# mahdi-slh/DeformContact

Measured on NVIDIA B200. Metric: train_step_graphs_per_sec, higher is better.
Workload: dtype fp32

## Files before the change

### deformcontact_b200/csrc/gemm_tc2.cu

```cuda
#include <cuda.h>
#include <stdlib.h>
#include <string.h>

#include <vector>

#include "common.cuh"

namespace dcb {
namespace {

constexpr int T2_BM = 128, T2_BN = 128, T2_BK = 32;
constexpr int T2_STAGES = 3;
constexpr int T2_THREADS = 512;
constexpr int T2_TILE_BYTES = T2_BM * T2_BK * 4;
constexpr int T2_STAGE_BYTES = 4 * T2_TILE_BYTES;
constexpr int T2_EPI_ROW = 20;
constexpr int T2_EPI_WARP_FLOATS = 32 * T2_EPI_ROW;
constexpr int T2_SMEM_BYTES = T2_STAGES * T2_STAGE_BYTES + 8 * T2_EPI_WARP_FLOATS * 4 + 256 + 1024;
constexpr int T2_DRAIN_KB = 4;
constexpr int T2_DRAIN_KB_SHORT = 4;
constexpr int T2_SHORT_KB = 16;
constexpr int T2_PART_KB = 8;
constexpr int T2_MAX_KPARTS = 64;

struct alignas(64) T2Problem {
  CUtensorMap mapA, mapB;
  CUtensorMap mapC, mapE;
  float* C;
  long long ldc;
  int M, N, kb_total, n_chunks;
  const float* E;
  const float* rowv;
  long long lde;
  int pad[2];
};

struct T2Params {
  const T2Problem* batch;
  const int* item_off;
  int n_problems;
  int nseg;
  int kb_seg[4];
  int kb_total;
  int M, N;
  int m_tiles, n_chunks, k_parts, kb_per_part, items;
  int a_mn, b_mn;
  int drain_kb;
  float* C;
  long long ldc;
  const float* bias;
  int relu, accumulate;
  float* partial;
  int pair;
  int raw_hi;
  int lo_rn;
  float comp;
  int tepi;
};

__device__ __forceinline__ uint32_t smem_u32(const void* p) { return (uint32_t)__cvta_generic_to_shared(p); }
__device__ __forceinline__ void mbar_init(uint32_t bar, uint32_t count) {
  asm volatile("mbarrier.init.shared::cta.b64 [%0], %1;" ::"r"(bar), "r"(count));
}
__device__ __forceinline__ void mbar_arrive(uint32_t bar) {
  asm volatile("mbarrier.arrive.shared::cta.b64 _, [%0];" ::"r"(bar) : "memory");
}
__device__ __forceinline__ void mbar_expect_tx(uint32_t bar, uint32_t bytes) {
  asm volatile("mbarrier.arrive.expect_tx.shared::cta.b64 _, [%0], %1;" ::"r"(bar), "r"(bytes) : "memory");
}
__device__ __forceinline__ void mbar_wait(uint32_t bar, uint32_t parity) {
  asm volatile(
      "{\n\t"
      ".reg .pred p;\n\t"
      "WAIT_%=:\n\t"
      "mbarrier.try_wait.parity.shared::cta.b64 p, [%0], %1;\n\t"
      "@p bra DONE_%=;\n\t"
      "bra WAIT_%=;\n\t"
      "DONE_%=:\n\t"
      "}" ::"r"(bar), "r"(parity)
      : "memory");
}
__device__ __forceinline__ void tma_load_2d(uint32_t dst, const CUtensorMap* map, uint32_t bar, int c0, int c1) {
  asm volatile(
      "cp.async.bulk.tensor.2d.shared::cluster.global.mbarrier::complete_tx::bytes [%0], [%1, {%3, %4}], [%2];" ::"r"(dst),
      "l"(map), "r"(bar), "r"(c0), "r"(c1)
      : "memory");
}
__device__ __forceinline__ void tma_store_2d(const CUtensorMap* map, uint32_t src, int c0, int c1) {
  asm volatile("cp.async.bulk.tensor.2d.global.shared::cta.bulk_group [%0, {%2, %3}], [%1];" ::"l"(map), "r"(src), "r"(c0), "r"(c1)
               : "memory");
}
__device__ __forceinline__ uint64_t l2_evict_first_policy() {
  uint64_t pol;
  asm volatile("createpolicy.fractional.L2::evict_first.b64 %0, 1.0;" : "=l"(pol));
  return pol;
}
__device__ __forceinline__ void tma_store_2d_hint(const CUtensorMap* map, uint32_t src, int c0, int c1, uint64_t pol) {
  asm volatile("cp.async.bulk.tensor.2d.global.shared::cta.bulk_group.L2::cache_hint [%0, {%2, %3}], [%1], %4;" ::"l"(map), "r"(src),
               "r"(c0), "r"(c1), "l"(pol)
               : "memory");
}
__device__ __forceinline__ void tma_load_2d_hint(uint32_t dst, const CUtensorMap* map, uint32_t bar, int c0, int c1, uint64_t pol) {
  asm volatile(
      "cp.async.bulk.tensor.2d.shared::cluster.global.mbarrier::complete_tx::bytes.L2::cache_hint [%0], [%1, {%3, %4}], [%2], %5;" ::"r"(dst),
      "l"(map), "r"(bar), "r"(c0), "r"(c1), "l"(pol)
      : "memory");
}
__device__ __forceinline__ void bulk_commit() { asm volatile("cp.async.bulk.commit_group;" ::: "memory"); }
__device__ __forceinline__ void bulk_wait_read0() { asm volatile("cp.async.bulk.wait_group.read 0;" ::: "memory"); }
__device__ __forceinline__ void bulk_wait0() { asm volatile("cp.async.bulk.wait_group 0;" ::: "memory"); }
__device__ __forceinline__ void tensormap_acquire(const CUtensorMap* map) {
  asm volatile("fence.proxy.tensormap::generic.acquire.sys [%0], 128;" ::"l"(map) : "memory");
}
__device__ __forceinline__ void umma_tf32(uint32_t d_tmem, uint64_t adesc, uint64_t bdesc, uint32_t idesc, uint32_t accum) {
  asm volatile(
      "{\n\t"
      ".reg .pred p;\n\t"
      "setp.ne.b32 p, %4, 0;\n\t"
      "tcgen05.mma.cta_group::1.kind::tf32 [%0], %1, %2, %3, p;\n\t"
      "}" ::"r"(d_tmem),
      "l"(adesc), "l"(bdesc), "r"(idesc), "r"(accum)
      : "memory");
}
__device__ __forceinline__ void umma_commit(uint32_t bar) {
  asm volatile("tcgen05.commit.cta_group::1.mbarrier::arrive::one.shared::cluster.b64 [%0];" ::"r"(bar) : "memory");
}
__device__ __forceinline__ uint32_t cluster_ctarank() {
  uint32_t r;
  asm volatile("mov.u32 %0, %%cluster_ctarank;" : "=r"(r));
  return r;
}
__device__ __forceinline__ void cluster_sync_all() {
  asm volatile("barrier.cluster.arrive.release.aligned;" ::: "memory");
  asm volatile("barrier.cluster.wait.acquire.aligned;" ::: "memory");
  __syncthreads();
}
__device__ __forceinline__ void mbar_arrive_rank(uint32_t bar, uint32_t rank) {
  uint32_t remote;
  asm volatile("mapa.shared::cluster.u32 %0, %1, %2;" : "=r"(remote) : "r"(bar), "r"(rank));
  asm volatile("mbarrier.arrive.shared::cluster.b64 _, [%0];" ::"r"(remote) : "memory");
}
__device__ __forceinline__ void umma2_tf32(uint32_t d_tmem, uint64_t adesc, uint64_t bdesc, uint32_t idesc, uint32_t accum) {
  asm volatile(
      "{\n\t"
      ".reg .pred p;\n\t"
      "setp.ne.b32 p, %4, 0;\n\t"
      "tcgen05.mma.cta_group::2.kind::tf32 [%0], %1, %2, %3, p;\n\t"
      "}" ::"r"(d_tmem),
      "l"(adesc), "l"(bdesc), "r"(idesc), "r"(accum)
      : "memory");
}
__device__ __forceinline__ void umma_commit2(uint32_t bar) {
  asm volatile("tcgen05.commit.cta_group::2.mbarrier::arrive::one.shared::cluster.multicast::cluster.b64 [%0], %1;" ::"r"(bar),
               "h"((unsigned short)3)
               : "memory");
}
__device__ __forceinline__ void tc_fence_before() { asm volatile("tcgen05.fence::before_thread_sync;" ::: "memory"); }
__device__ __forceinline__ void tc_fence_after() { asm volatile("tcgen05.fence::after_thread_sync;" ::: "memory"); }

__device__ __forceinline__ uint64_t desc_kmajor(uint32_t saddr) {
  uint64_t d = 0;
  d |= (uint64_t)((saddr & 0x3FFFF) >> 4);
  d |= (uint64_t)1 << 16;
  d |= (uint64_t)(1024 >> 4) << 32;
  d |= (uint64_t)1 << 46;
  d |= (uint64_t)2 << 61;
  return d;
}
__device__ __forceinline__ uint64_t desc_mnmajor(uint32_t saddr) {
  uint64_t d = 0;
  d |= (uint64_t)((saddr & 0x3FFFF) >> 4);
  d |= (uint64_t)((4096 >> 4) & 0x3FFF) << 16;
  d |= (uint64_t)((512 >> 4) & 0x3FFF) << 32;
  d |= (uint64_t)1 << 46;
  d |= (uint64_t)1 << 61;
  return d;
}

#define T2_TMEM_LD32(R, ADDR)                                                                                            \
  asm volatile(                                                                                                         \
      "tcgen05.ld.sync.aligned.32x32b.x32.b32 "                                                                         \
      "{%0, %1, %2, %3, %4, %5, %6, %7, %8, %9, %10, %11, %12, %13, %14, %15, %16, %17, %18, %19, %20, %21, %22, %23, " \
      "%24, %25, %26, %27, %28, %29, %30, %31}, [%32];"                                                                 \
      : "=r"(R[0]), "=r"(R[1]), "=r"(R[2]), "=r"(R[3]), "=r"(R[4]), "=r"(R[5]), "=r"(R[6]), "=r"(R[7]), "=r"(R[8]),    \
        "=r"(R[9]), "=r"(R[10]), "=r"(R[11]), "=r"(R[12]), "=r"(R[13]), "=r"(R[14]), "=r"(R[15]), "=r"(R[16]),         \
        "=r"(R[17]), "=r"(R[18]), "=r"(R[19]), "=r"(R[20]), "=r"(R[21]), "=r"(R[22]), "=r"(R[23]), "=r"(R[24]),        \
        "=r"(R[25]), "=r"(R[26]), "=r"(R[27]), "=r"(R[28]), "=r"(R[29]), "=r"(R[30]), "=r"(R[31])                       \
      : "r"(ADDR))

struct T2Item {
  int m0, n0, part, kb0, kb1;
  int M, N;
  float* C;
  long long ldc;
  const CUtensorMap *mapA, *mapB;
  const CUtensorMap *mapC, *mapE;
  const float *E, *rowv;
  long long lde;
};
__device__ __forceinline__ T2Item t2_item(const T2Params& p, int w, int& pidx, int rank = 0) {
  T2Item it;
  if (p.batch) {
    while (w >= p.item_off[pidx + 1]) ++pidx;
    const T2Problem* q = p.batch + pidx;
    const int local = w - p.item_off[pidx];
    const int nch = q->n_chunks;
    it.part = 0;
    it.n0 = (local % nch) * T2_BN;
    it.m0 = (p.pair ? (local / nch) * 2 + rank : (local / nch)) * T2_BM;
    it.kb0 = 0;
    it.kb1 = q->kb_total;
    it.M = q->M; it.N = q->N; it.C = q->C; it.ldc = q->ldc;
    it.mapA = &q->mapA; it.mapB = &q->mapB;
    it.mapC = &q->mapC; it.mapE = &q->mapE;
    it.E = q->E; it.rowv = q->rowv; it.lde = q->lde;
    return it;
  }
  it.part = w % p.k_parts;
  const int mn = w / p.k_parts;
  it.n0 = (mn % p.n_chunks) * T2_BN;
  it.m0 = (p.pair ? (mn / p.n_chunks) * 2 + rank : (mn / p.n_chunks)) * T2_BM;
  it.kb0 = it.part * p.kb_per_part;
  it.kb1 = min(p.kb_total, it.kb0 + p.kb_per_part);
  it.M = p.M; it.N = p.N; it.C = p.C; it.ldc = p.ldc;
  it.mapA = nullptr; it.mapB = nullptr;
  it.mapC = nullptr; it.mapE = nullptr;
  it.E = nullptr; it.rowv = nullptr; it.lde = 0;
  return it;
}

template <bool PAIR, bool TEPI>
__global__ void __launch_bounds__(T2_THREADS, 1)
gemm_tc2_kernel(const __grid_constant__ CUtensorMap mapA0, const __grid_constant__ CUtensorMap mapA1,
                const __grid_constant__ CUtensorMap mapA2, const __grid_constant__ CUtensorMap mapA3,
                const __grid_constant__ CUtensorMap mapB0, const __grid_constant__ CUtensorMap mapB1,
                const __grid_constant__ CUtensorMap mapB2, const __grid_constant__ CUtensorMap mapB3,
                const __grid_constant__ CUtensorMap mapC0, const T2Params p) {
  static_assert(PAIR || !TEPI, "the TMA epilogue exists for CTA pairs only");
  extern __shared__ uint8_t smem_raw[];
  const uint32_t base = (smem_u32(smem_raw) + 1023u) & ~1023u;
  uint8_t* base_ptr = smem_raw + (base - smem_u32(smem_raw));
  constexpr int NST = PAIR ? (TEPI ? 3 : 4) : T2_STAGES;
  constexpr int STB = PAIR ? 3 * T2_TILE_BYTES : T2_STAGE_BYTES;
  constexpr int RING = NST * STB;
  constexpr int EPI_WARP_BYTES = TEPI ? 8192 : T2_EPI_WARP_FLOATS * 4;
  constexpr int B_OFF = 2 * T2_TILE_BYTES;
  constexpr int BLO_OFF = PAIR ? B_OFF + T2_TILE_BYTES / 2 : B_OFF + T2_TILE_BYTES;
  static_assert(RING + 8 * EPI_WARP_BYTES + 256 + 1024 <= T2_SMEM_BYTES, "shared memory carve");
  static_assert(TEPI || RING == T2_STAGES * T2_STAGE_BYTES, "stage ring size");
  float* epi_stage = reinterpret_cast<float*>(base_ptr + RING);
  const uint32_t bar_base = base + RING + 8 * EPI_WARP_BYTES;
  auto ebar = [&](int slot) { return bar_base + 160u + 8u * slot; };
  auto full_bar = [&](int s) { return bar_base + 8u * s; };
  auto xform_bar = [&](int s) { return bar_base + 32u + 8u * s; };
  auto empty_bar = [&](int s) { return bar_base + 64u + 8u * s; };
  auto tfull_bar = [&](int j) { return bar_base + 96u + 8u * j; };
  auto tempty_bar = [&](int j) { return bar_base + 112u + 8u * j; };
  volatile uint32_t* tmem_ptr_smem = reinterpret_cast<volatile uint32_t*>(base_ptr + RING + 8 * EPI_WARP_BYTES + 144);

  const int warp = threadIdx.x >> 5, lane = threadIdx.x & 31;
  const int rank = PAIR ? (int)cluster_ctarank() : 0;
  const int w0 = PAIR ? (int)(blockIdx.x >> 1) : (int)blockIdx.x;
  const int wstep = PAIR ? (int)(gridDim.x >> 1) : (int)gridDim.x;

  if (threadIdx.x == 0) {
    for (int s = 0; s < NST; ++s) {
      mbar_init(full_bar(s), 1);
      mbar_init(xform_bar(s), PAIR ? 8 : 128);
      mbar_init(empty_bar(s), 1);
    }
    for (int j = 0; j < 2; ++j) {
      mbar_init(tfull_bar(j), 1);
      mbar_init(tempty_bar(j), PAIR ? 16 : 256);
    }
    if (TEPI)
      for (int sl = 0; sl < 8; ++sl) mbar_init(ebar(sl), 1);
    asm volatile("fence.mbarrier_init.release.cluster;" ::: "memory");
  }
  if (warp == 2) {
    if (PAIR) {
      asm volatile("tcgen05.alloc.cta_group::2.sync.aligned.shared::cta.b32 [%0], %1;" ::"r"(smem_u32((const void*)tmem_ptr_smem)),
                   "r"(512u)
                   : "memory");
      asm volatile("tcgen05.relinquish_alloc_permit.cta_group::2.sync.aligned;" ::: "memory");
    } else {
      asm volatile("tcgen05.alloc.cta_group::1.sync.aligned.shared::cta.b32 [%0], %1;" ::"r"(smem_u32((const void*)tmem_ptr_smem)),
                   "r"(512u)
                   : "memory");
      asm volatile("tcgen05.relinquish_alloc_permit.cta_group::1.sync.aligned;" ::: "memory");
    }
  }
  tc_fence_before();
  if (PAIR) cluster_sync_all(); else __syncthreads();
  tc_fence_after();
  const uint32_t tmem_base = *tmem_ptr_smem;

  if (warp == 0) {
    if (lane == 0) {
      const CUtensorMap* mA[4] = {&mapA0, &mapA1, &mapA2, &mapA3};
      const CUtensorMap* mB[4] = {&mapB0, &mapB1, &mapB2, &mapB3};
      int it = 0, pidx = 0, fenced = -1;
      for (int w = w0; w < p.items; w += wstep) {
        const T2Item item = t2_item(p, w, pidx, rank);
        if (p.batch) {
          mA[0] = item.mapA; mB[0] = item.mapB;
          if (fenced != pidx) {
            tensormap_acquire(item.mapA);
            tensormap_acquire(item.mapB);
            fenced = pidx;
          }
        }
        int seg = 0, seg_kb0 = 0;
        for (int kb = item.kb0; kb < item.kb1; ++kb, ++it) {
          if (!p.batch)
            while (kb >= seg_kb0 + p.kb_seg[seg]) { seg_kb0 += p.kb_seg[seg]; ++seg; }
          const int k0 = (kb - seg_kb0) * T2_BK;
          const int st = it % NST;
          const uint32_t ph = (it / NST) & 1;
          mbar_wait(empty_bar(st), ph ^ 1);
          const uint32_t sbase = base + st * STB;
          mbar_expect_tx(full_bar(st), PAIR ? T2_TILE_BYTES + T2_TILE_BYTES / 2 : 2 * T2_TILE_BYTES);
          if (p.a_mn) {
#pragma unroll
            for (int c = 0; c < 4; ++c) tma_load_2d(sbase + c * 4096, mA[seg], full_bar(st), item.m0 + c * 32, k0);
          } else {
            tma_load_2d(sbase, mA[seg], full_bar(st), k0, item.m0);
          }
          if (PAIR) {
            const int nb0 = item.n0 + rank * (T2_BN / 2);
            if (p.b_mn) {
#pragma unroll
              for (int c = 0; c < 2; ++c) tma_load_2d(sbase + 2 * T2_TILE_BYTES + c * 4096, mB[seg], full_bar(st), nb0 + c * 32, k0);
            } else {
              tma_load_2d(sbase + 2 * T2_TILE_BYTES, mB[seg], full_bar(st), k0, nb0);
            }
          } else if (p.b_mn) {
#pragma unroll
            for (int c = 0; c < 4; ++c) tma_load_2d(sbase + 2 * T2_TILE_BYTES + c * 4096, mB[seg], full_bar(st), item.n0 + c * 32, k0);
          } else {
            tma_load_2d(sbase + 2 * T2_TILE_BYTES, mB[seg], full_bar(st), k0, item.n0);
          }
        }
      }
    }
  } else if (warp == 1) {
    if (lane == 0 && rank == 0) {
      const uint32_t idesc = (1u << 4) | (2u << 7) | (2u << 10) | ((uint32_t)p.a_mn << 15) | ((uint32_t)p.b_mn << 16) |
                             ((uint32_t)(T2_BN >> 3) << 17) | ((uint32_t)(T2_BM >> 4) << 24);
      const uint32_t a_adv = p.a_mn ? (1024u >> 4) : (32u >> 4), b_adv = p.b_mn ? (1024u >> 4) : (32u >> 4);
      const uint32_t idesc256 = (idesc & ~(0x3Fu << 17)) | ((uint32_t)(2 * T2_BN >> 3) << 17);
      const uint32_t idesc_pair = (idesc & ~(0x1Fu << 24)) | ((uint32_t)(2 * T2_BM >> 4) << 24);
      int it = 0, chain = 0, pidx = 0;
      for (int w = w0; w < p.items; w += wstep) {
        const T2Item item = t2_item(p, w, pidx, rank);
        for (int kc0 = item.kb0; kc0 < item.kb1; kc0 += p.drain_kb, ++chain) {
          const int kc1 = min(item.kb1, kc0 + p.drain_kb);
          const int j = chain & 1;
          const uint32_t d_main = tmem_base + (uint32_t)(2 * T2_BN * j), d_cross = d_main + (uint32_t)T2_BN;
          mbar_wait(tempty_bar(j), ((chain >> 1) & 1) ^ 1);
          tc_fence_after();
          for (int kb = kc0; kb < kc1; ++kb, ++it) {
            const int st = it % NST;
            const uint32_t ph = (it / NST) & 1;
            mbar_wait(full_bar(st), ph);
            mbar_wait(xform_bar(st), ph);
            tc_fence_after();
            const uint32_t sbase = base + st * STB;
            const uint64_t a_hi = p.a_mn ? desc_mnmajor(sbase) : desc_kmajor(sbase);
            const uint64_t a_lo = p.a_mn ? desc_mnmajor(sbase + T2_TILE_BYTES) : desc_kmajor(sbase + T2_TILE_BYTES);
            const uint64_t b_hi = p.b_mn ? desc_mnmajor(sbase + 2 * T2_TILE_BYTES) : desc_kmajor(sbase + 2 * T2_TILE_BYTES);
            if (PAIR) {
              const uint64_t b_lo = p.b_mn ? desc_mnmajor(sbase + BLO_OFF) : desc_kmajor(sbase + BLO_OFF);
#pragma unroll
              for (int kk = 0; kk < T2_BK / 8; ++kk) {
                const uint64_t aa = (uint64_t)(kk * a_adv), bb = (uint64_t)(kk * b_adv);
                const uint32_t acc = (kb > kc0 || kk > 0) ? 1u : 0u;
                umma2_tf32(d_main, a_hi + aa, b_hi + bb, idesc_pair, acc);
                umma2_tf32(d_cross, a_hi + aa, b_lo + bb, idesc_pair, acc);
                umma2_tf32(d_cross, a_lo + aa, b_hi + bb, idesc_pair, 1u);
              }
              umma_commit2(empty_bar(st));
            } else {
#pragma unroll
            for (int kk = 0; kk < T2_BK / 8; ++kk) {
              const uint64_t aa = (uint64_t)(kk * a_adv), bb = (uint64_t)(kk * b_adv);
              const uint32_t acc = (kb > kc0 || kk > 0) ? 1u : 0u;
              umma_tf32(d_main, a_hi + aa, b_hi + bb, idesc256, acc);
              umma_tf32(d_cross, a_lo + aa, b_hi + bb, idesc, 1u);
            }
            umma_commit(empty_bar(st));
            }
          }
          if (PAIR) umma_commit2(tfull_bar(j)); else umma_commit(tfull_bar(j));
        }
      }
    }
  } else if (warp >= 8 && warp < 12) {
    const int t = threadIdx.x - 256;
    const uint32_t rb = p.lo_rn ? 0x1000u : 0u;
    int it = 0, pidx = 0;
    for (int w = w0; w < p.items; w += wstep) {
      const T2Item item = t2_item(p, w, pidx, rank);
      for (int kb = item.kb0; kb < item.kb1; ++kb, ++it) {
        const int st = it % NST;
        const uint32_t ph = (it / NST) & 1;
        mbar_wait(full_bar(st), ph);
        uint4* a = reinterpret_cast<uint4*>(base_ptr + st * STB);
        uint4* b = reinterpret_cast<uint4*>(base_ptr + st * STB + B_OFF);
        constexpr int LO = T2_TILE_BYTES / 16;
        constexpr int LO_B = (BLO_OFF - B_OFF) / 16;
#pragma unroll
        for (int i = 0; i < 2 * T2_TILE_BYTES / 16 / 128; ++i) {
          if (PAIR && (i & 1) && (i >> 1) >= T2_TILE_BYTES / 32 / 128) continue;
          uint4* src = (i & 1) ? b : a;
          const int idx = t + (i >> 1) * 128;
          const uint4 v = src[idx];
          const uint4 h = make_uint4(v.x & 0xFFFFE000u, v.y & 0xFFFFE000u, v.z & 0xFFFFE000u, v.w & 0xFFFFE000u);
          uint4 l;
          l.x = __float_as_uint(__uint_as_float(v.x) - __uint_as_float(h.x)) + rb;
          l.y = __float_as_uint(__uint_as_float(v.y) - __uint_as_float(h.y)) + rb;
          l.z = __float_as_uint(__uint_as_float(v.z) - __uint_as_float(h.z)) + rb;
          l.w = __float_as_uint(__uint_as_float(v.w) - __uint_as_float(h.w)) + rb;
          if (!p.raw_hi) src[idx] = h;
          src[idx + ((i & 1) ? LO_B : LO)] = l;
        }
        asm volatile("fence.proxy.async.shared::cta;" ::: "memory");
        if (PAIR) {
          __syncwarp();
          if (lane == 0) mbar_arrive_rank(xform_bar(st), 0);
        } else {
          mbar_arrive(xform_bar(st));
        }
      }
    }
  } else if (warp >= 4) {
    const int q = warp & 3;
    const int half = warp >= 12 ? 1 : 0;
    float* stg = epi_stage + ((half * 4) + q) * T2_EPI_WARP_FLOATS;
    const uint32_t lane_addr = tmem_base + ((uint32_t)(q * 32) << 16) + (uint32_t)(half * 64);
    int chain = 0, pidx = 0;
    const int slot = half * 4 + q;
    const uint32_t ebuf = base + RING + slot * 8192;
    uint8_t* ebuf_ptr = base_ptr + RING + slot * 8192;
    uint32_t eph = 0;
    int efenced = -1;
    const bool ehint = TEPI && (p.tepi & 2);
    const uint64_t epol = ehint ? l2_evict_first_policy() : 0ull;
    for (int w = w0; w < p.items; w += wstep) {
      const T2Item item = t2_item(p, w, pidx, rank);
      const bool vec_ok = ((item.ldc & 3) == 0) && ((reinterpret_cast<uintptr_t>(item.C) & 15) == 0) &&
                          (!p.bias || (reinterpret_cast<uintptr_t>(p.bias) & 15) == 0) && ((item.N & 3) == 0 || p.k_parts == 1);
      float acc[64];
#pragma unroll
      for (int i = 0; i < 64; ++i) acc[i] = 0.f;
      const CUtensorMap* mC = TEPI ? (p.batch ? item.mapC : &mapC0) : nullptr;
      const int ecol0 = item.n0 + half * 64, erow0 = item.m0 + q * 32;
      if (TEPI) {
        if (lane == 0) {
          bulk_wait_read0();
          if (p.batch && efenced != pidx) {
            tensormap_acquire(item.mapC);
            if (item.E != nullptr) tensormap_acquire(item.mapE);
            efenced = pidx;
          }
          if (item.E != nullptr) {
            mbar_expect_tx(ebar(slot), 8192);
            if (ehint) {
              tma_load_2d_hint(ebuf, item.mapE, ebar(slot), ecol0, erow0, epol);
              tma_load_2d_hint(ebuf + 4096, item.mapE, ebar(slot), ecol0 + 32, erow0, epol);
            } else {
              tma_load_2d(ebuf, item.mapE, ebar(slot), ecol0, erow0);
              tma_load_2d(ebuf + 4096, item.mapE, ebar(slot), ecol0 + 32, erow0);
            }
          }
        }
        __syncwarp();
      }
      if (!TEPI && item.E != nullptr) {
        auto prefetch_block = [&](const T2Item& it2) {
          const int prow = it2.m0 + q * 32 + lane;
          const int pcol = it2.n0 + half * 64;
          if (it2.E != nullptr && prow < it2.M && pcol < it2.N) {
            const float* pe = it2.E + (long long)prow * it2.lde + pcol;
            asm volatile("prefetch.global.L2 [%0];" ::"l"(pe));
            if (pcol + 32 < it2.N) asm volatile("prefetch.global.L2 [%0];" ::"l"(pe + 32));
            if (pcol + 63 < it2.N) asm volatile("prefetch.global.L2 [%0];" ::"l"(pe + 63));
          }
        };
        if (w == w0) prefetch_block(item);
        if (w + wstep < p.items) {
          int pidx2 = pidx;
          prefetch_block(t2_item(p, w + wstep, pidx2, rank));
        }
      }
      for (int kc0 = item.kb0; kc0 < item.kb1; kc0 += p.drain_kb, ++chain) {
        const int j = chain & 1;
        mbar_wait(tfull_bar(j), (chain >> 1) & 1);
        tc_fence_after();
        const uint32_t cbase = lane_addr + (uint32_t)(2 * T2_BN * j);
        const float comp = 1.0f + p.comp * (float)(4 * (min(item.kb1, kc0 + p.drain_kb) - kc0));
        uint32_t r[32];
#pragma unroll
        for (int part = 0; part < 4; ++part) {
          T2_TMEM_LD32(r, cbase + (uint32_t)((part >> 1) * T2_BN + (part & 1) * 32));
          asm volatile("tcgen05.wait::ld.sync.aligned;" ::: "memory");
          if (part == 3) {
            tc_fence_before();
            if (PAIR) {
              __syncwarp();
              if (lane == 0) mbar_arrive_rank(tempty_bar(j), 0);
            } else {
              mbar_arrive(tempty_bar(j));
            }
          }
          if (part < 2) {
#pragma unroll
            for (int i = 0; i < 32; ++i) acc[(part & 1) * 32 + i] = fmaf(__uint_as_float(r[i]), comp, acc[(part & 1) * 32 + i]);
          } else {
#pragma unroll
            for (int i = 0; i < 32; ++i) acc[(part & 1) * 32 + i] += __uint_as_float(r[i]);
          }
        }
      }
      if (TEPI) {
        const int row = erow0 + lane;
        float d = 0.f;
        if (item.E != nullptr) {
          if (row < item.M) d = __ldg(item.rowv + row);
          mbar_wait(ebar(slot), eph);
          eph ^= 1;
        }
        const float* bias = p.bias;
        const bool bias_vec = bias && ((reinterpret_cast<uintptr_t>(bias) & 15) == 0);
#pragma unroll
        for (int b = 0; b < 2; ++b) {
#pragma unroll
          for (int c = 0; c < 8; ++c) {
            float4* cell = reinterpret_cast<float4*>(ebuf_ptr + b * 4096 + lane * 128 + ((c ^ (lane & 7)) << 4));
            float4 v = make_float4(acc[b * 32 + c * 4], acc[b * 32 + c * 4 + 1], acc[b * 32 + c * 4 + 2], acc[b * 32 + c * 4 + 3]);
            if (bias) {
              const int col = ecol0 + b * 32 + c * 4;
              if (bias_vec && col + 3 < item.N) {
                const float4 bv = __ldg(reinterpret_cast<const float4*>(bias + col));
                v.x += bv.x; v.y += bv.y; v.z += bv.z; v.w += bv.w;
              } else {
                if (col < item.N) v.x += __ldg(bias + col);
                if (col + 1 < item.N) v.y += __ldg(bias + col + 1);
                if (col + 2 < item.N) v.z += __ldg(bias + col + 2);
                if (col + 3 < item.N) v.w += __ldg(bias + col + 3);
              }
            }
            if (item.E != nullptr) {
              const float4 e = *cell;
              v.x = e.x * (v.x - d); v.y = e.y * (v.y - d); v.z = e.z * (v.z - d); v.w = e.w * (v.w - d);
            }
            if (p.relu) { v.x = fmaxf(v.x, 0.f); v.y = fmaxf(v.y, 0.f); v.z = fmaxf(v.z, 0.f); v.w = fmaxf(v.w, 0.f); }
            *cell = v;
          }
        }
        asm volatile("fence.proxy.async.shared::cta;" ::: "memory");
        __syncwarp();
        if (lane == 0) {
          if (ehint) {
            tma_store_2d_hint(mC, ebuf, ecol0, erow0, epol);
            tma_store_2d_hint(mC, ebuf + 4096, ecol0 + 32, erow0, epol);
          } else {
            tma_store_2d(mC, ebuf, ecol0, erow0);
            tma_store_2d(mC, ebuf + 4096, ecol0 + 32, erow0);
          }
          bulk_commit();
        }
        continue;
      }
      const bool to_slab = p.k_parts > 1;
      float* outp = to_slab ? p.partial + (size_t)item.part * (size_t)item.M * item.N : item.C;
      const long long ldo = to_slab ? (long long)item.N : item.ldc;
      const bool add_c = !to_slab && p.accumulate;
      const bool do_relu = !to_slab && p.relu;
      const float* bias = to_slab ? nullptr : p.bias;
      const int row0 = item.m0 + q * 32;
      if (item.E != nullptr && vec_ok && !add_c && !do_relu && !bias && (item.N & 3) == 0 && (item.lde & 3) == 0 &&
          (reinterpret_cast<uintptr_t>(item.E) & 15) == 0) {
        const int c4 = (lane >> 3) * 4;
        const int rsub = lane & 7;
        const int colbase = item.n0 + half * 64 + c4;
        const float* erow = item.E + (long long)(row0 + rsub) * item.lde + colbase;
        float* orow = outp + (long long)(row0 + rsub) * ldo + colbase;
        float4 xa[4], xb[4];
        float dv[4];
#pragma unroll
        for (int it4 = 0; it4 < 4; ++it4) dv[it4] = (row0 + it4 * 8 + rsub < item.M) ? __ldg(item.rowv + row0 + it4 * 8 + rsub) : 0.f;
        auto load_group = [&](float4 (&x)[4], int g) {
#pragma unroll
          for (int it4 = 0; it4 < 4; ++it4) {
            x[it4] = make_float4(0.f, 0.f, 0.f, 0.f);
            if (row0 + it4 * 8 + rsub < item.M && colbase + g * 16 < item.N)
              x[it4] = __ldcs(reinterpret_cast<const float4*>(erow + (long long)(it4 * 8) * item.lde + g * 16));
          }
        };
        load_group(xa, 0);
#pragma unroll
        for (int g = 0; g < 4; ++g) {
#pragma unroll
          for (int jv = 0; jv < 16; jv += 4)
            *reinterpret_cast<float4*>(stg + lane * T2_EPI_ROW + jv) = make_float4(acc[g * 16 + jv], acc[g * 16 + jv + 1], acc[g * 16 + jv + 2], acc[g * 16 + jv + 3]);
          __syncwarp();
          if (g + 1 < 4) { if (g & 1) load_group(xa, g + 1); else load_group(xb, g + 1); }
#pragma unroll
          for (int it4 = 0; it4 < 4; ++it4) {
            const int rr = it4 * 8 + rsub;
            if (row0 + rr < item.M && colbase + g * 16 < item.N) {
              float4 v = *reinterpret_cast<const float4*>(stg + rr * T2_EPI_ROW + c4);
              const float4 e = (g & 1) ? xb[it4] : xa[it4];
              const float d = dv[it4];
              v.x = e.x * (v.x - d); v.y = e.y * (v.y - d); v.z = e.z * (v.z - d); v.w = e.w * (v.w - d);
              __stcs(reinterpret_cast<float4*>(orow + (long long)(it4 * 8) * ldo + g * 16), v);
            }
          }
          __syncwarp();
        }
        continue;
      }
#pragma unroll
      for (int g = 0; g < 4; ++g) {
#pragma unroll
        for (int jv = 0; jv < 16; jv += 4)
          *reinterpret_cast<float4*>(stg + lane * T2_EPI_ROW + jv) = make_float4(acc[g * 16 + jv], acc[g * 16 + jv + 1], acc[g * 16 + jv + 2], acc[g * 16 + jv + 3]);
        __syncwarp();
        const int c4 = (lane >> 3) * 4;
        const int col = item.n0 + half * 64 + g * 16 + c4;
        if (vec_ok && col + 3 < item.N) {
          const float4 bv = bias ? *reinterpret_cast<const float4*>(bias + col) : make_float4(0.f, 0.f, 0.f, 0.f);
#pragma unroll
          for (int it4 = 0; it4 < 4; ++it4) {
            const int rr = it4 * 8 + (lane & 7);
            const int row = row0 + rr;
            if (row < item.M) {
              float4 v = *reinterpret_cast<const float4*>(stg + rr * T2_EPI_ROW + c4);
              v.x += bv.x; v.y += bv.y; v.z += bv.z; v.w += bv.w;
              if (item.E) {
                const float d = item.rowv[row];
                const float* ep = item.E + (long long)row * item.lde + col;
                float4 e4;
                if (((item.lde & 3) == 0) && ((reinterpret_cast<uintptr_t>(item.E) & 15) == 0)) e4 = *reinterpret_cast<const float4*>(ep);
                else e4 = make_float4(ep[0], ep[1], ep[2], ep[3]);
                v.x = e4.x * (v.x - d); v.y = e4.y * (v.y - d); v.z = e4.z * (v.z - d); v.w = e4.w * (v.w - d);
              }
              float4* dst = reinterpret_cast<float4*>(outp + (long long)row * ldo + col);
              if (add_c) { const float4 o = *dst; v.x += o.x; v.y += o.y; v.z += o.z; v.w += o.w; }
              if (do_relu) { v.x = fmaxf(v.x, 0.f); v.y = fmaxf(v.y, 0.f); v.z = fmaxf(v.z, 0.f); v.w = fmaxf(v.w, 0.f); }
              *dst = v;
            }
          }
        } else {
          for (int it4 = 0; it4 < 4; ++it4) {
            const int rr = it4 * 8 + (lane & 7);
            const int row = row0 + rr;
            for (int e = 0; e < 4; ++e) {
              if (row < item.M && col + e < item.N) {
                float v = stg[rr * T2_EPI_ROW + c4 + e] + (bias ? bias[col + e] : 0.f);
                if (item.E) v = item.E[(long long)row * item.lde + col + e] * (v - item.rowv[row]);
                float* dst = outp + (long long)row * ldo + col + e;
                if (add_c) v += *dst;
                if (do_relu) v = fmaxf(v, 0.f);
                *dst = v;
              }
            }
          }
        }
        __syncwarp();
      }
    }
  }

  if (TEPI && warp >= 4 && !(warp >= 8 && warp < 12) && lane == 0) bulk_wait0();
  tc_fence_before();
  if (PAIR) cluster_sync_all(); else __syncthreads();
  if (warp == 2) {
    tc_fence_after();
    if (PAIR) asm volatile("tcgen05.dealloc.cta_group::2.sync.aligned.b32 %0, %1;" ::"r"(tmem_base), "r"(512u) : "memory");
    else asm volatile("tcgen05.dealloc.cta_group::1.sync.aligned.b32 %0, %1;" ::"r"(tmem_base), "r"(512u) : "memory");
  }
}

__global__ void t2_reduce_kernel(const float* __restrict__ partial, int parts, long long MN, int N, float* __restrict__ C,
                                 long long ldc, const float* __restrict__ bias, int relu, int accumulate) {
  const long long idx = blockIdx.x * (long long)blockDim.x + threadIdx.x;
  if (idx >= MN) return;
  const long long m = idx / N;
  const int n = (int)(idx % N);
  float s = 0.f;
  for (int z = 0; z < parts; ++z) s += partial[(size_t)z * MN + idx];
  if (bias) s += bias[n];
  float* dst = C + m * ldc + n;
  if (accumulate) s += *dst;
  if (relu) s = fmaxf(s, 0.f);
  *dst = s;
}

typedef CUresult (*EncodeFn2)(CUtensorMap*, CUtensorMapDataType, cuuint32_t, void*, const cuuint64_t*, const cuuint64_t*,
                              const cuuint32_t*, const cuuint32_t*, CUtensorMapInterleave, CUtensorMapSwizzle,
                              CUtensorMapL2promotion, CUtensorMapFloatOOBfill);
EncodeFn2 get_encode2() {
  static EncodeFn2 fn = nullptr;
  if (!fn) {
    void* sym = nullptr;
    cudaDriverEntryPointQueryResult qres;
    if (cudaGetDriverEntryPoint("cuTensorMapEncodeTiled", &sym, cudaEnableDefault, &qres) == cudaSuccess &&
        qres == cudaDriverEntryPointSuccess)
      fn = reinterpret_cast<EncodeFn2>(sym);
  }
  return fn;
}

int make_map2(CUtensorMap* map, const float* ptr, uint64_t inner, uint64_t rows, uint64_t ld_elems, uint32_t box_rows,
              CUtensorMapSwizzle swz) {
  EncodeFn2 enc = get_encode2();
  DC_REQUIRE(enc, DC_ECUDA, "gemm_tc2: cuTensorMapEncodeTiled not available");
  cuuint64_t gdim[2] = {inner, rows};
  cuuint64_t gstr[1] = {ld_elems * 4};
  cuuint32_t box[2] = {T2_BK, box_rows};
  cuuint32_t estr[2] = {1, 1};
  CUresult r = enc(map, CU_TENSOR_MAP_DATA_TYPE_FLOAT32, 2, const_cast<float*>(ptr), gdim, gstr, box, estr,
                   CU_TENSOR_MAP_INTERLEAVE_NONE, swz, CU_TENSOR_MAP_L2_PROMOTION_L2_128B, CU_TENSOR_MAP_FLOAT_OOB_FILL_NONE);
  DC_REQUIRE(r == CUDA_SUCCESS, DC_ECUDA, "gemm_tc2: cuTensorMapEncodeTiled failed (%d)", (int)r);
  return DC_OK;
}

int t2_drain_kb(int64_t kb_total) {
  static int d_long = -1, d_short = -1;
  if (d_long < 0) {
    const char* e = getenv("DCB200_DRAIN_KB");
    d_long = (e && atoi(e) > 0) ? atoi(e) : T2_DRAIN_KB;
    const char* es = getenv("DCB200_DRAIN_KB_SHORT");
    d_short = (es && atoi(es) > 0) ? atoi(es) : T2_DRAIN_KB_SHORT;
  }
  return kb_total <= T2_SHORT_KB ? (d_short < d_long ? d_short : d_long) : d_long;
}

void t2_numerics(T2Params& p) {
  static int lo_rn = -1;
  static float comp = -1.f;
  if (lo_rn < 0) {
    const char* e = getenv("DCB200_T2_LO_RN");
    lo_rn = e ? (e[0] == '1') : 1;
    const char* c = getenv("DCB200_T2_COMP");
    comp = c ? (float)atof(c) : 2.6e-8f;
  }
  p.lo_rn = lo_rn;
  p.comp = comp;
}

int t2_pair() {
  static int pair = -1;
  if (pair < 0) {
    const char* e = getenv("DCB200_T2_PAIR");
    pair = e ? (e[0] == '1') : 1;
  }
  return pair;
}

int t2_tepi_mode() {
  static int mode = -1;
  if (mode < 0) {
    const char* e = getenv("DCB200_T2_TEPI");
    mode = e ? atoi(e) : 3;
  }
  return mode;
}
bool t2_tepi_ok(int pair, int64_t kb_max, int k_parts, int accumulate) {
  const int mode = t2_tepi_mode();
  return pair && mode > 0 && k_parts == 1 && !accumulate && (mode > 1 || kb_max <= T2_SHORT_KB);
}
bool t2_tepi_operand_ok(const float* ptr, int64_t ld) { return ptr && (ld & 3) == 0 && (reinterpret_cast<uintptr_t>(ptr) & 15) == 0; }

int t2_launch(const CUtensorMap* mA, const CUtensorMap* mB, const CUtensorMap& mC, const T2Params& p, cudaStream_t st) {
  static DeviceOnce attr_set;
  if (attr_set.first()) {
    DC_CUDA(cudaFuncSetAttribute(gemm_tc2_kernel<false, false>, cudaFuncAttributeMaxDynamicSharedMemorySize, T2_SMEM_BYTES));
    DC_CUDA(cudaFuncSetAttribute(gemm_tc2_kernel<true, false>, cudaFuncAttributeMaxDynamicSharedMemorySize, T2_SMEM_BYTES));
    DC_CUDA(cudaFuncSetAttribute(gemm_tc2_kernel<true, true>, cudaFuncAttributeMaxDynamicSharedMemorySize, T2_SMEM_BYTES));
  }
  if (!p.pair) {
    const int grid = p.items < sm_count() ? p.items : sm_count();
    gemm_tc2_kernel<false, false><<<grid, T2_THREADS, T2_SMEM_BYTES, st>>>(mA[0], mA[1], mA[2], mA[3], mB[0], mB[1], mB[2], mB[3], mC, p);
  } else {
    const int pairs = p.items < sm_count() / 2 ? p.items : sm_count() / 2;
    cudaLaunchConfig_t cfg{};
    cfg.gridDim = dim3((unsigned)(2 * pairs));
    cfg.blockDim = dim3(T2_THREADS);
    cfg.dynamicSmemBytes = T2_SMEM_BYTES;
    cfg.stream = st;
    cudaLaunchAttribute at[1];
    at[0].id = cudaLaunchAttributeClusterDimension;
    at[0].val.clusterDim.x = 2; at[0].val.clusterDim.y = 1; at[0].val.clusterDim.z = 1;
    cfg.attrs = at;
    cfg.numAttrs = 1;
    if (p.tepi) DC_CUDA(cudaLaunchKernelEx(&cfg, gemm_tc2_kernel<true, true>, mA[0], mA[1], mA[2], mA[3], mB[0], mB[1], mB[2], mB[3], mC, p));
    else DC_CUDA(cudaLaunchKernelEx(&cfg, gemm_tc2_kernel<true, false>, mA[0], mA[1], mA[2], mA[3], mB[0], mB[1], mB[2], mB[3], mC, p));
  }
  DC_LAUNCH_CHECK();
  return DC_OK;
}

int t2_k_parts(int64_t M, int64_t N, int64_t kb_total) {
  const int64_t mn = cdiv(M, T2_BM) * cdiv(N, T2_BN);
  if (mn >= sm_count()) return 1;
  int64_t parts = sm_count() / mn;
  const int64_t max_parts = kb_total / T2_PART_KB;
  if (parts > max_parts) parts = max_parts;
  if (parts > T2_MAX_KPARTS) parts = T2_MAX_KPARTS;
  return parts < 1 ? 1 : (int)parts;
}
}

bool gemm_tc2_supported(const dc_gemm_seg* segs, int nseg, int transA, int transB, int64_t M, int64_t N) {
  if (nseg < 1 || nseg > 4 || M < 1 || N < 1 || M >= (1ll << 31) || N >= (1ll << 31)) return false;
  if (nseg > 1 && (transA || !transB)) return false;
  for (int s = 0; s < nseg; ++s) {
    if (segs[s].K <= 0 || segs[s].K >= (1ll << 31)) return false;
    if (segs[s].lda % 4 != 0 || segs[s].ldb % 4 != 0) return false;
    if ((reinterpret_cast<uintptr_t>(segs[s].A) & 15) || (reinterpret_cast<uintptr_t>(segs[s].B) & 15)) return false;
  }
  return true;
}

size_t gemm_tc2_workspace_bytes(int64_t M, int64_t N, int64_t Ktot) {
  const int parts = t2_k_parts(M, N, cdiv(Ktot, T2_BK));
  return parts > 1 ? align_up((size_t)parts * M * N * sizeof(float), 256) + 256 : 0;
}

int gemm_tc2(const dc_gemm_seg* segs, int nseg, int transA, int transB, int64_t M, int64_t N, float* C, int64_t ldc,
             const float* bias, int relu, int accumulate, void* workspace, size_t workspace_bytes, cudaStream_t st) {
  DC_REQUIRE(gemm_tc2_supported(segs, nseg, transA, transB, M, N), DC_ENOSUP, "gemm_tc2: layout not supported by the tcgen05 path");
  T2Params p{};
  p.nseg = nseg;
  p.a_mn = transA ? 1 : 0;
  p.b_mn = transB ? 0 : 1;
  p.pair = t2_pair();
  const uint32_t b_box_rows = p.pair ? T2_BN / 2 : T2_BN;
  CUtensorMap mA[4], mB[4];
  int64_t ktot = 0;
  for (int s = 0; s < 4; ++s) {
    const int ss = s < nseg ? s : 0;
    const uint64_t K = (uint64_t)segs[ss].K;
    if (transA) {
      if (int rc = make_map2(&mA[s], segs[ss].A, (uint64_t)M, K, (uint64_t)segs[ss].lda, 32, CU_TENSOR_MAP_SWIZZLE_128B_ATOM_32B)) return rc;
    } else {
      if (int rc = make_map2(&mA[s], segs[ss].A, K, (uint64_t)M, (uint64_t)segs[ss].lda, T2_BM, CU_TENSOR_MAP_SWIZZLE_128B)) return rc;
    }
    if (transB) {
      if (int rc = make_map2(&mB[s], segs[ss].B, K, (uint64_t)N, (uint64_t)segs[ss].ldb, b_box_rows, CU_TENSOR_MAP_SWIZZLE_128B)) return rc;
    } else {
      if (int rc = make_map2(&mB[s], segs[ss].B, (uint64_t)N, K, (uint64_t)segs[ss].ldb, 32, CU_TENSOR_MAP_SWIZZLE_128B_ATOM_32B)) return rc;
    }
    p.kb_seg[s] = s < nseg ? (int)cdiv(segs[s].K, T2_BK) : (1 << 30);
    if (s < nseg) ktot += cdiv(segs[s].K, T2_BK);
  }
  p.kb_total = (int)ktot;
  p.M = (int)M; p.N = (int)N;
  p.m_tiles = (int)cdiv(M, T2_BM);
  p.n_chunks = (int)cdiv(N, T2_BN);
  p.k_parts = t2_k_parts(M, N, p.kb_total);
  p.kb_per_part = (int)(cdiv(cdiv(p.kb_total, p.k_parts), T2_PART_KB) * T2_PART_KB);
  p.k_parts = (int)cdiv(p.kb_total, p.kb_per_part);
  p.items = (p.pair ? (p.m_tiles + 1) / 2 : p.m_tiles) * p.n_chunks * p.k_parts;
  p.drain_kb = t2_drain_kb(p.kb_total);
  p.C = C; p.ldc = ldc; p.bias = bias; p.relu = relu; p.accumulate = accumulate;
  p.raw_hi = 1;
  if (const char* e = getenv("DCB200_T2_RAWHI")) p.raw_hi = e[0] == '1';
  t2_numerics(p);
  if (p.k_parts > 1) {
    const size_t need = align_up((size_t)p.k_parts * M * N * sizeof(float), 256) + 256;
    DC_REQUIRE(workspace && workspace_bytes >= need, DC_EWORKSPACE, "gemm_tc2: workspace %zu < %zu", workspace_bytes, need);
    p.partial = reinterpret_cast<float*>((reinterpret_cast<uintptr_t>(workspace) + 255) & ~(uintptr_t)255);
  }
  CUtensorMap mC{};
  p.tepi = t2_tepi_ok(p.pair, p.kb_total, p.k_parts, accumulate) && t2_tepi_operand_ok(C, ldc);
  if (p.tepi)
    if (int rc = make_map2(&mC, C, (uint64_t)N, (uint64_t)M, (uint64_t)ldc, 32, CU_TENSOR_MAP_SWIZZLE_128B)) return rc;
  if (int rc = t2_launch(mA, mB, mC, p, st)) return rc;
  if (p.k_parts > 1) {
    const long long MN = (long long)M * N;
    t2_reduce_kernel<<<(unsigned)cdiv(MN, 256), 256, 0, st>>>(p.partial, p.k_parts, MN, (int)N, C, ldc, bias, relu, accumulate);
    DC_LAUNCH_CHECK();
  }
  return DC_OK;
}

size_t gemm_tc2_batched_workspace_bytes(int count) {
  if (count < 0) count = 0;
  return align_up((size_t)count * sizeof(T2Problem), 256) + align_up((size_t)(count + 1) * sizeof(int), 256) + 512;
}

int gemm_tc2_batched(const dc_gemm_problem* probs, int count, int transA, int transB, int relu, int accumulate, void* workspace,
                     size_t workspace_bytes, void* host_staging, size_t host_staging_bytes, cudaStream_t st) {
  DC_REQUIRE(probs && count > 0, DC_EINVAL, "gemm_batched: no problems");
  const size_t need = gemm_tc2_batched_workspace_bytes(count);
  DC_REQUIRE(workspace && workspace_bytes >= need, DC_EWORKSPACE, "gemm_batched: workspace %zu < %zu", workspace_bytes, need);
  const size_t tab_bytes = align_up((size_t)count * sizeof(T2Problem), 256);
  const size_t off_bytes = (size_t)(count + 1) * sizeof(int);
  std::vector<unsigned char> host;
  unsigned char* hraw = static_cast<unsigned char*>(host_staging);
  if (hraw) {
    DC_REQUIRE(host_staging_bytes >= tab_bytes + off_bytes + 64, DC_EWORKSPACE, "gemm_batched: host staging %zu < %zu",
               host_staging_bytes, tab_bytes + off_bytes + 64);
  } else {
    host.resize(tab_bytes + off_bytes + 64);
    hraw = host.data();
  }
  unsigned char* hbase = reinterpret_cast<unsigned char*>((reinterpret_cast<uintptr_t>(hraw) + 63) & ~(uintptr_t)63);
  T2Problem* tab = reinterpret_cast<T2Problem*>(hbase);
  int* item_off = reinterpret_cast<int*>(hbase + tab_bytes);
  const int pair = t2_pair();
  const uint32_t b_box_rows = pair ? T2_BN / 2 : T2_BN;
  int64_t items = 0;
  int64_t max_kb = 0;
  int64_t kb_all = 0;
  bool tepi_operands = true;
  for (int i = 0; i < count; ++i) {
    const dc_gemm_problem& q = probs[i];
    if (q.M <= 0 || q.N <= 0) continue;
    if (cdiv(q.K, T2_BK) > kb_all) kb_all = cdiv(q.K, T2_BK);
    if (!t2_tepi_operand_ok(q.C, q.ldc) || (q.E && !t2_tepi_operand_ok(q.E, q.lde))) tepi_operands = false;
  }
  bool any_e = false;
  for (int i = 0; i < count; ++i) any_e = any_e || probs[i].E != nullptr;
  const int tepi = t2_tepi_ok(pair, kb_all, 1, accumulate) && tepi_operands && (t2_tepi_mode() != 3 || any_e);
  for (int i = 0; i < count; ++i) {
    const dc_gemm_problem& q = probs[i];
    DC_REQUIRE(q.M >= 0 && q.N >= 0 && q.K >= 0, DC_EINVAL, "gemm_batched: negative size in problem %d", i);
    item_off[i] = (int)items;
    T2Problem& t = tab[i];
    memset(&t, 0, sizeof(t));
    if (q.M == 0 || q.N == 0) continue;
    DC_REQUIRE(q.K > 0, DC_ENOSUP, "gemm_batched: K = 0 in problem %d (zero the output instead)", i);
    dc_gemm_seg seg{q.A, q.lda, q.B, q.ldb, q.K};
    DC_REQUIRE(gemm_tc2_supported(&seg, 1, transA, transB, q.M, q.N) && q.C && q.ldc >= q.N, DC_ENOSUP,
               "gemm_batched: problem %d is not supported by the tcgen05 path (needs lda/ldb %% 4 == 0, 16-byte aligned operands)", i);
    if (transA) {
      if (int rc = make_map2(&t.mapA, q.A, (uint64_t)q.M, (uint64_t)q.K, (uint64_t)q.lda, 32, CU_TENSOR_MAP_SWIZZLE_128B_ATOM_32B)) return rc;
    } else {
      if (int rc = make_map2(&t.mapA, q.A, (uint64_t)q.K, (uint64_t)q.M, (uint64_t)q.lda, T2_BM, CU_TENSOR_MAP_SWIZZLE_128B)) return rc;
    }
    if (transB) {
      if (int rc = make_map2(&t.mapB, q.B, (uint64_t)q.K, (uint64_t)q.N, (uint64_t)q.ldb, b_box_rows, CU_TENSOR_MAP_SWIZZLE_128B)) return rc;
    } else {
      if (int rc = make_map2(&t.mapB, q.B, (uint64_t)q.N, (uint64_t)q.K, (uint64_t)q.ldb, 32, CU_TENSOR_MAP_SWIZZLE_128B_ATOM_32B)) return rc;
    }
    t.C = q.C; t.ldc = q.ldc; t.M = (int)q.M; t.N = (int)q.N;
    t.E = q.E; t.rowv = q.rowv; t.lde = q.lde;
    DC_REQUIRE(!q.E || (q.rowv && q.lde >= q.N), DC_EINVAL, "gemm_batched: problem %d: epilogue operand needs rowv and lde >= N", i);
    if (tepi) {
      if (int rc = make_map2(&t.mapC, q.C, (uint64_t)q.N, (uint64_t)q.M, (uint64_t)q.ldc, 32, CU_TENSOR_MAP_SWIZZLE_128B)) return rc;
      if (q.E)
        if (int rc = make_map2(&t.mapE, q.E, (uint64_t)q.N, (uint64_t)q.M, (uint64_t)q.lde, 32, CU_TENSOR_MAP_SWIZZLE_128B)) return rc;
    }
    t.kb_total = (int)cdiv(q.K, T2_BK);
    if (t.kb_total > max_kb) max_kb = t.kb_total;
    t.n_chunks = (int)cdiv(q.N, T2_BN);
    items += (pair ? cdiv(cdiv(q.M, T2_BM), 2) : cdiv(q.M, T2_BM)) * t.n_chunks;
    DC_REQUIRE(items < (1ll << 30), DC_ENOSUP, "gemm_batched: too many work items");
  }
  item_off[count] = (int)items;
  if (items == 0) return DC_OK;
  unsigned char* dbase = reinterpret_cast<unsigned char*>((reinterpret_cast<uintptr_t>(workspace) + 255) & ~(uintptr_t)255);
  DC_CUDA(cudaMemcpyAsync(dbase, hbase, tab_bytes + off_bytes, cudaMemcpyHostToDevice, st));
  T2Params p{};
  p.batch = reinterpret_cast<const T2Problem*>(dbase);
  p.item_off = reinterpret_cast<const int*>(dbase + tab_bytes);
  p.n_problems = count;
  p.nseg = 1;
  p.kb_seg[0] = 1 << 30;
  p.a_mn = transA ? 1 : 0;
  p.b_mn = transB ? 0 : 1;
  p.k_parts = 1;
  p.pair = pair;
  p.items = (int)items;
  p.drain_kb = t2_drain_kb(max_kb);
  p.relu = relu; p.accumulate = accumulate;
  p.raw_hi = 1;
  if (const char* e = getenv("DCB200_T2_RAWHI")) p.raw_hi = e[0] == '1';
  t2_numerics(p);
  static int hint = -1;
  if (hint < 0) { const char* e = getenv("DCB200_T2_TEPI_HINT"); hint = e ? atoi(e) : 1; }
  p.tepi = tepi ? (hint ? 3 : 1) : 0;
  CUtensorMap dummy[4]{};
  return t2_launch(dummy, dummy, dummy[0], p, st);
}

}
```

Before: 2822.

## Add wide 256-column CTA-pair GEMM tiles with warp-specialized register split

Adds a WIDE kernel variant in which each CTA pair computes a 256x256 output tile: every CTA loads a full 128-row B tile and the MMA uses N=256 instruction descriptors that fill all of TMEM in a single buffer. setmaxnreg shifts registers from the producer and transform warps to the epilogue warps, which read TMEM in x16 chunks. The goal is to halve A-tile reloads and per-item overhead when N exceeds 128 and there are enough items. In exchange TMEM is no longer double-buffered, so the epilogue and the next MMA chain overlap less, and the TMA epilogue and E-operand fusion are turned off on this path.

```diff
diff --git a/deformcontact_b200/csrc/gemm_tc2.cu b/deformcontact_b200/csrc/gemm_tc2.cu
--- a/deformcontact_b200/csrc/gemm_tc2.cu
+++ b/deformcontact_b200/csrc/gemm_tc2.cu
@@ -22,6 +22,8 @@
 constexpr int T2_SHORT_KB = 16;
 constexpr int T2_PART_KB = 8;
 constexpr int T2_MAX_KPARTS = 64;
+constexpr int T2_WIDE_REGS_WG0 = 56, T2_WIDE_REGS_SPLIT = 72, T2_WIDE_REGS_EPI = 192;
+static_assert(T2_WIDE_REGS_WG0 + T2_WIDE_REGS_SPLIT + 2 * T2_WIDE_REGS_EPI == 4 * (65536 / T2_THREADS), "register file split");
 
 struct alignas(64) T2Problem {
   CUtensorMap mapA, mapB;
@@ -56,6 +58,7 @@
   int lo_rn;
   float comp;
   int tepi;
+  int wide;
 };
 
 __device__ __forceinline__ uint32_t smem_u32(const void* p) { return (uint32_t)__cvta_generic_to_shared(p); }
@@ -188,6 +191,14 @@
         "=r"(R[25]), "=r"(R[26]), "=r"(R[27]), "=r"(R[28]), "=r"(R[29]), "=r"(R[30]), "=r"(R[31])                       \
       : "r"(ADDR))
 
+#define T2_TMEM_LD16(R, ADDR)                                                                                            \
+  asm volatile(                                                                                                         \
+      "tcgen05.ld.sync.aligned.32x32b.x16.b32 "                                                                         \
+      "{%0, %1, %2, %3, %4, %5, %6, %7, %8, %9, %10, %11, %12, %13, %14, %15}, [%16];"                                  \
+      : "=r"(R[0]), "=r"(R[1]), "=r"(R[2]), "=r"(R[3]), "=r"(R[4]), "=r"(R[5]), "=r"(R[6]), "=r"(R[7]), "=r"(R[8]),    \
+        "=r"(R[9]), "=r"(R[10]), "=r"(R[11]), "=r"(R[12]), "=r"(R[13]), "=r"(R[14]), "=r"(R[15])                        \
+      : "r"(ADDR))
+
 struct T2Item {
   int m0, n0, part, kb0, kb1;
   int M, N;
@@ -198,6 +209,7 @@
   const float *E, *rowv;
   long long lde;
 };
+template <bool WIDE>
 __device__ __forceinline__ T2Item t2_item(const T2Params& p, int w, int& pidx, int rank = 0) {
   T2Item it;
   if (p.batch) {
@@ -206,7 +218,7 @@
     const int local = w - p.item_off[pidx];
     const int nch = q->n_chunks;
     it.part = 0;
-    it.n0 = (local % nch) * T2_BN;
+    it.n0 = (local % nch) * (WIDE ? 2 * T2_BN : T2_BN);
     it.m0 = (p.pair ? (local / nch) * 2 + rank : (local / nch)) * T2_BM;
     it.kb0 = 0;
     it.kb1 = q->kb_total;
@@ -218,7 +230,7 @@
   }
   it.part = w % p.k_parts;
   const int mn = w / p.k_parts;
-  it.n0 = (mn % p.n_chunks) * T2_BN;
+  it.n0 = (mn % p.n_chunks) * (WIDE ? 2 * T2_BN : T2_BN);
   it.m0 = (p.pair ? (mn / p.n_chunks) * 2 + rank : (mn / p.n_chunks)) * T2_BM;
   it.kb0 = it.part * p.kb_per_part;
   it.kb1 = min(p.kb_total, it.kb0 + p.kb_per_part);
@@ -229,7 +241,7 @@
   return it;
 }
 
-template <bool PAIR, bool TEPI>
+template <bool PAIR, bool TEPI, bool WIDE>
 __global__ void __launch_bounds__(T2_THREADS, 1)
 gemm_tc2_kernel(const __grid_constant__ CUtensorMap mapA0, const __grid_constant__ CUtensorMap mapA1,
                 const __grid_constant__ CUtensorMap mapA2, const __grid_constant__ CUtensorMap mapA3,
@@ -237,15 +249,18 @@
                 const __grid_constant__ CUtensorMap mapB2, const __grid_constant__ CUtensorMap mapB3,
                 const __grid_constant__ CUtensorMap mapC0, const T2Params p) {
   static_assert(PAIR || !TEPI, "the TMA epilogue exists for CTA pairs only");
+  static_assert(!WIDE || (PAIR && !TEPI), "wide items exist for CTA pairs with the staged epilogue only");
   extern __shared__ uint8_t smem_raw[];
   const uint32_t base = (smem_u32(smem_raw) + 1023u) & ~1023u;
   uint8_t* base_ptr = smem_raw + (base - smem_u32(smem_raw));
-  constexpr int NST = PAIR ? (TEPI ? 3 : 4) : T2_STAGES;
-  constexpr int STB = PAIR ? 3 * T2_TILE_BYTES : T2_STAGE_BYTES;
+  constexpr bool HALF_B = PAIR && !WIDE;
+  constexpr int NST = HALF_B ? (TEPI ? 3 : 4) : T2_STAGES;
+  constexpr int STB = HALF_B ? 3 * T2_TILE_BYTES : T2_STAGE_BYTES;
+  constexpr int B_ROWS = HALF_B ? T2_BN / 2 : T2_BN;
   constexpr int RING = NST * STB;
   constexpr int EPI_WARP_BYTES = TEPI ? 8192 : T2_EPI_WARP_FLOATS * 4;
   constexpr int B_OFF = 2 * T2_TILE_BYTES;
-  constexpr int BLO_OFF = PAIR ? B_OFF + T2_TILE_BYTES / 2 : B_OFF + T2_TILE_BYTES;
+  constexpr int BLO_OFF = B_OFF + B_ROWS * T2_BK * 4;
   static_assert(RING + 8 * EPI_WARP_BYTES + 256 + 1024 <= T2_SMEM_BYTES, "shared memory carve");
   static_assert(TEPI || RING == T2_STAGES * T2_STAGE_BYTES, "stage ring size");
   float* epi_stage = reinterpret_cast<float*>(base_ptr + RING);
@@ -295,112 +310,125 @@
   tc_fence_after();
   const uint32_t tmem_base = *tmem_ptr_smem;
 
-  if (warp == 0) {
-    if (lane == 0) {
-      const CUtensorMap* mA[4] = {&mapA0, &mapA1, &mapA2, &mapA3};
-      const CUtensorMap* mB[4] = {&mapB0, &mapB1, &mapB2, &mapB3};
-      int it = 0, pidx = 0, fenced = -1;
-      for (int w = w0; w < p.items; w += wstep) {
-        const T2Item item = t2_item(p, w, pidx, rank);
-        if (p.batch) {
-          mA[0] = item.mapA; mB[0] = item.mapB;
-          if (fenced != pidx) {
-            tensormap_acquire(item.mapA);
-            tensormap_acquire(item.mapB);
-            fenced = pidx;
-          }
-        }
-        int seg = 0, seg_kb0 = 0;
-        for (int kb = item.kb0; kb < item.kb1; ++kb, ++it) {
-          if (!p.batch)
-            while (kb >= seg_kb0 + p.kb_seg[seg]) { seg_kb0 += p.kb_seg[seg]; ++seg; }
-          const int k0 = (kb - seg_kb0) * T2_BK;
-          const int st = it % NST;
-          const uint32_t ph = (it / NST) & 1;
-          mbar_wait(empty_bar(st), ph ^ 1);
-          const uint32_t sbase = base + st * STB;
-          mbar_expect_tx(full_bar(st), PAIR ? T2_TILE_BYTES + T2_TILE_BYTES / 2 : 2 * T2_TILE_BYTES);
-          if (p.a_mn) {
-#pragma unroll
-            for (int c = 0; c < 4; ++c) tma_load_2d(sbase + c * 4096, mA[seg], full_bar(st), item.m0 + c * 32, k0);
-          } else {
-            tma_load_2d(sbase, mA[seg], full_bar(st), k0, item.m0);
-          }
-          if (PAIR) {
-            const int nb0 = item.n0 + rank * (T2_BN / 2);
-            if (p.b_mn) {
-#pragma unroll
-              for (int c = 0; c < 2; ++c) tma_load_2d(sbase + 2 * T2_TILE_BYTES + c * 4096, mB[seg], full_bar(st), nb0 + c * 32, k0);
-            } else {
-              tma_load_2d(sbase + 2 * T2_TILE_BYTES, mB[seg], full_bar(st), k0, nb0);
+  if (warp < 4) {
+    if (WIDE) asm volatile("setmaxnreg.dec.sync.aligned.u32 %0;" ::"n"(T2_WIDE_REGS_WG0));
+    if (warp == 0) {
+      if (lane == 0) {
+        int it = 0, pidx = 0, fenced = -1;
+        for (int w = w0; w < p.items; w += wstep) {
+          const T2Item item = t2_item<WIDE>(p, w, pidx, rank);
+          if (p.batch) {
+            if (fenced != pidx) {
+              tensormap_acquire(item.mapA);
+              tensormap_acquire(item.mapB);
+              fenced = pidx;
             }
-          } else if (p.b_mn) {
-#pragma unroll
-            for (int c = 0; c < 4; ++c) tma_load_2d(sbase + 2 * T2_TILE_BYTES + c * 4096, mB[seg], full_bar(st), item.n0 + c * 32, k0);
-          } else {
-            tma_load_2d(sbase + 2 * T2_TILE_BYTES, mB[seg], full_bar(st), k0, item.n0);
-          }
-        }
-      }
-    }
-  } else if (warp == 1) {
-    if (lane == 0 && rank == 0) {
-      const uint32_t idesc = (1u << 4) | (2u << 7) | (2u << 10) | ((uint32_t)p.a_mn << 15) | ((uint32_t)p.b_mn << 16) |
-                             ((uint32_t)(T2_BN >> 3) << 17) | ((uint32_t)(T2_BM >> 4) << 24);
-      const uint32_t a_adv = p.a_mn ? (1024u >> 4) : (32u >> 4), b_adv = p.b_mn ? (1024u >> 4) : (32u >> 4);
-      const uint32_t idesc256 = (idesc & ~(0x3Fu << 17)) | ((uint32_t)(2 * T2_BN >> 3) << 17);
-      const uint32_t idesc_pair = (idesc & ~(0x1Fu << 24)) | ((uint32_t)(2 * T2_BM >> 4) << 24);
-      int it = 0, chain = 0, pidx = 0;
-      for (int w = w0; w < p.items; w += wstep) {
-        const T2Item item = t2_item(p, w, pidx, rank);
-        for (int kc0 = item.kb0; kc0 < item.kb1; kc0 += p.drain_kb, ++chain) {
-          const int kc1 = min(item.kb1, kc0 + p.drain_kb);
-          const int j = chain & 1;
-          const uint32_t d_main = tmem_base + (uint32_t)(2 * T2_BN * j), d_cross = d_main + (uint32_t)T2_BN;
-          mbar_wait(tempty_bar(j), ((chain >> 1) & 1) ^ 1);
-          tc_fence_after();
-          for (int kb = kc0; kb < kc1; ++kb, ++it) {
+          }
+          int seg = 0, seg_kb0 = 0;
+          for (int kb = item.kb0; kb < item.kb1; ++kb, ++it) {
+            if (!p.batch)
+              while (kb >= seg_kb0 + p.kb_seg[seg]) { seg_kb0 += p.kb_seg[seg]; ++seg; }
+            const int k0 = (kb - seg_kb0) * T2_BK;
+            const CUtensorMap* ma = p.batch ? item.mapA : seg == 0 ? &mapA0 : seg == 1 ? &mapA1 : seg == 2 ? &mapA2 : &mapA3;
+            const CUtensorMap* mb = p.batch ? item.mapB : seg == 0 ? &mapB0 : seg == 1 ? &mapB1 : seg == 2 ? &mapB2 : &mapB3;
             const int st = it % NST;
             const uint32_t ph = (it / NST) & 1;
-            mbar_wait(full_bar(st), ph);
-            mbar_wait(xform_bar(st), ph);
+            mbar_wait(empty_bar(st), ph ^ 1);
+            const uint32_t sbase = base + st * STB;
+            mbar_expect_tx(full_bar(st), T2_TILE_BYTES + B_ROWS * T2_BK * 4);
+            if (p.a_mn) {
+  #pragma unroll
+              for (int c = 0; c < 4; ++c) tma_load_2d(sbase + c * 4096, ma, full_bar(st), item.m0 + c * 32, k0);
+            } else {
+              tma_load_2d(sbase, ma, full_bar(st), k0, item.m0);
+            }
+            const int nb0 = item.n0 + rank * B_ROWS;
+            if (p.b_mn) {
+  #pragma unroll
+              for (int c = 0; c < B_ROWS / 32; ++c) tma_load_2d(sbase + 2 * T2_TILE_BYTES + c * 4096, mb, full_bar(st), nb0 + c * 32, k0);
+            } else {
+              tma_load_2d(sbase + 2 * T2_TILE_BYTES, mb, full_bar(st), k0, nb0);
+            }
+          }
+        }
+      }
+    } else if (warp == 1) {
+      if (lane == 0 && rank == 0) {
+        const uint32_t idesc = (1u << 4) | (2u << 7) | (2u << 10) | ((uint32_t)p.a_mn << 15) | ((uint32_t)p.b_mn << 16) |
+                               ((uint32_t)(T2_BN >> 3) << 17) | ((uint32_t)(T2_BM >> 4) << 24);
+        const uint32_t a_adv = p.a_mn ? (1024u >> 4) : (32u >> 4), b_adv = p.b_mn ? (1024u >> 4) : (32u >> 4);
+        const uint32_t idesc256 = (idesc & ~(0x3Fu << 17)) | ((uint32_t)(2 * T2_BN >> 3) << 17);
+        const uint32_t idesc_pair = (idesc & ~(0x1Fu << 24)) | ((uint32_t)(2 * T2_BM >> 4) << 24);
+        const uint32_t idesc_wide = (idesc_pair & ~(0x3Fu << 17)) | ((uint32_t)(2 * T2_BN >> 3) << 17);
+        int it = 0, chain = 0, pidx = 0;
+        for (int w = w0; w < p.items; w += wstep) {
+          const T2Item item = t2_item<WIDE>(p, w, pidx, rank);
+          for (int kc0 = item.kb0; kc0 < item.kb1; kc0 += p.drain_kb, ++chain) {
+            const int kc1 = min(item.kb1, kc0 + p.drain_kb);
+            const int j = WIDE ? 0 : chain & 1;
+            const uint32_t d_main = tmem_base + (uint32_t)(2 * T2_BN * j), d_cross = d_main + (uint32_t)(WIDE ? 2 * T2_BN : T2_BN);
+            const uint32_t tph = WIDE ? (chain & 1) ^ 1 : ((chain >> 1) & 1) ^ 1;
+            mbar_wait(tempty_bar(j), tph);
             tc_fence_after();
-            const uint32_t sbase = base + st * STB;
-            const uint64_t a_hi = p.a_mn ? desc_mnmajor(sbase) : desc_kmajor(sbase);
-            const uint64_t a_lo = p.a_mn ? desc_mnmajor(sbase + T2_TILE_BYTES) : desc_kmajor(sbase + T2_TILE_BYTES);
-            const uint64_t b_hi = p.b_mn ? desc_mnmajor(sbase + 2 * T2_TILE_BYTES) : desc_kmajor(sbase + 2 * T2_TILE_BYTES);
-            if (PAIR) {
-              const uint64_t b_lo = p.b_mn ? desc_mnmajor(sbase + BLO_OFF) : desc_kmajor(sbase + BLO_OFF);
-#pragma unroll
+            for (int kb = kc0; kb < kc1; ++kb, ++it) {
+              const int st = it % NST;
+              const uint32_t ph = (it / NST) & 1;
+              mbar_wait(full_bar(st), ph);
+              mbar_wait(xform_bar(st), ph);
+              tc_fence_after();
+              const uint32_t sbase = base + st * STB;
+              const uint64_t a_hi = p.a_mn ? desc_mnmajor(sbase) : desc_kmajor(sbase);
+              const uint64_t a_lo = p.a_mn ? desc_mnmajor(sbase + T2_TILE_BYTES) : desc_kmajor(sbase + T2_TILE_BYTES);
+              const uint64_t b_hi = p.b_mn ? desc_mnmajor(sbase + 2 * T2_TILE_BYTES) : desc_kmajor(sbase + 2 * T2_TILE_BYTES);
+              if (WIDE) {
+                const uint64_t b_lo = p.b_mn ? desc_mnmajor(sbase + BLO_OFF) : desc_kmajor(sbase + BLO_OFF);
+  #pragma unroll
+                for (int kk = 0; kk < T2_BK / 8; ++kk) {
+                  const uint64_t aa = (uint64_t)(kk * a_adv), bb = (uint64_t)(kk * b_adv);
+                  const uint32_t acc = (kb > kc0 || kk > 0) ? 1u : 0u;
+                  umma2_tf32(d_main, a_hi + aa, b_hi + bb, idesc_wide, acc);
+                  if (!acc) {
+                    mbar_wait(tempty_bar(1), tph);
+                    tc_fence_after();
+                  }
+                  umma2_tf32(d_cross, a_hi + aa, b_lo + bb, idesc_wide, acc);
+                  umma2_tf32(d_cross, a_lo + aa, b_hi + bb, idesc_wide, 1u);
+                }
+                umma_commit2(empty_bar(st));
+              } else if (PAIR) {
+                const uint64_t b_lo = p.b_mn ? desc_mnmajor(sbase + BLO_OFF) : desc_kmajor(sbase + BLO_OFF);
+  #pragma unroll
+                for (int kk = 0; kk < T2_BK / 8; ++kk) {
+                  const uint64_t aa = (uint64_t)(kk * a_adv), bb = (uint64_t)(kk * b_adv);
+                  const uint32_t acc = (kb > kc0 || kk > 0) ? 1u : 0u;
+                  umma2_tf32(d_main, a_hi + aa, b_hi + bb, idesc_pair, acc);
+                  umma2_tf32(d_cross, a_hi + aa, b_lo + bb, idesc_pair, acc);
+                  umma2_tf32(d_cross, a_lo + aa, b_hi + bb, idesc_pair, 1u);
+                }
+                umma_commit2(empty_bar(st));
+              } else {
+  #pragma unroll
               for (int kk = 0; kk < T2_BK / 8; ++kk) {
                 const uint64_t aa = (uint64_t)(kk * a_adv), bb = (uint64_t)(kk * b_adv);
                 const uint32_t acc = (kb > kc0 || kk > 0) ? 1u : 0u;
-                umma2_tf32(d_main, a_hi + aa, b_hi + bb, idesc_pair, acc);
-                umma2_tf32(d_cross, a_hi + aa, b_lo + bb, idesc_pair, acc);
-                umma2_tf32(d_cross, a_lo + aa, b_hi + bb, idesc_pair, 1u);
+                umma_tf32(d_main, a_hi + aa, b_hi + bb, idesc256, acc);
+                umma_tf32(d_cross, a_lo + aa, b_hi + bb, idesc, 1u);
               }
-              umma_commit2(empty_bar(st));
-            } else {
-#pragma unroll
-            for (int kk = 0; kk < T2_BK / 8; ++kk) {
-              const uint64_t aa = (uint64_t)(kk * a_adv), bb = (uint64_t)(kk * b_adv);
-              const uint32_t acc = (kb > kc0 || kk > 0) ? 1u : 0u;
-              umma_tf32(d_main, a_hi + aa, b_hi + bb, idesc256, acc);
-              umma_tf32(d_cross, a_lo + aa, b_hi + bb, idesc, 1u);
+              umma_commit(empty_bar(st));
+              }
             }
-            umma_commit(empty_bar(st));
-            }
-          }
-          if (PAIR) umma_commit2(tfull_bar(j)); else umma_commit(tfull_bar(j));
+            if (PAIR) umma_commit2(tfull_bar(j)); else umma_commit(tfull_bar(j));
+          }
         }
       }
     }
   } else if (warp >= 8 && warp < 12) {
+    if (WIDE) asm volatile("setmaxnreg.dec.sync.aligned.u32 %0;" ::"n"(T2_WIDE_REGS_SPLIT));
     const int t = threadIdx.x - 256;
     const uint32_t rb = p.lo_rn ? 0x1000u : 0u;
     int it = 0, pidx = 0;
     for (int w = w0; w < p.items; w += wstep) {
-      const T2Item item = t2_item(p, w, pidx, rank);
+      const T2Item item = t2_item<WIDE>(p, w, pidx, rank);
       for (int kb = item.kb0; kb < item.kb1; ++kb, ++it) {
         const int st = it % NST;
         const uint32_t ph = (it / NST) & 1;
@@ -411,7 +439,7 @@
         constexpr int LO_B = (BLO_OFF - B_OFF) / 16;
 #pragma unroll
         for (int i = 0; i < 2 * T2_TILE_BYTES / 16 / 128; ++i) {
-          if (PAIR && (i & 1) && (i >> 1) >= T2_TILE_BYTES / 32 / 128) continue;
+          if (HALF_B && (i & 1) && (i >> 1) >= T2_TILE_BYTES / 32 / 128) continue;
           uint4* src = (i & 1) ? b : a;
           const int idx = t + (i >> 1) * 128;
           const uint4 v = src[idx];
@@ -433,11 +461,15 @@
         }
       }
     }
-  } else if (warp >= 4) {
+  } else {
+    if (WIDE) asm volatile("setmaxnreg.inc.sync.aligned.u32 %0;" ::"n"(T2_WIDE_REGS_EPI));
+    constexpr int CW = WIDE ? T2_BN : T2_BN / 2;
+    constexpr int LDW = WIDE ? 16 : 32;
+    constexpr int NPART = 2 * CW / LDW;
     const int q = warp & 3;
     const int half = warp >= 12 ? 1 : 0;
     float* stg = epi_stage + ((half * 4) + q) * T2_EPI_WARP_FLOATS;
-    const uint32_t lane_addr = tmem_base + ((uint32_t)(q * 32) << 16) + (uint32_t)(half * 64);
+    const uint32_t lane_addr = tmem_base + ((uint32_t)(q * 32) << 16) + (uint32_t)(half * CW);
     int chain = 0, pidx = 0;
     const int slot = half * 4 + q;
     const uint32_t ebuf = base + RING + slot * 8192;
@@ -447,12 +479,12 @@
     const bool ehint = TEPI && (p.tepi & 2);
     const uint64_t epol = ehint ? l2_evict_first_policy() : 0ull;
     for (int w = w0; w < p.items; w += wstep) {
-      const T2Item item = t2_item(p, w, pidx, rank);
+      const T2Item item = t2_item<WIDE>(p, w, pidx, rank);
       const bool vec_ok = ((item.ldc & 3) == 0) && ((reinterpret_cast<uintptr_t>(item.C) & 15) == 0) &&
                           (!p.bias || (reinterpret_cast<uintptr_t>(p.bias) & 15) == 0) && ((item.N & 3) == 0 || p.k_parts == 1);
-      float acc[64];
-#pragma unroll
-      for (int i = 0; i < 64; ++i) acc[i] = 0.f;
+      float acc[CW];
+#pragma unroll
+      for (int i = 0; i < CW; ++i) acc[i] = 0.f;
       const CUtensorMap* mC = TEPI ? (p.batch ? item.mapC : &mapC0) : nullptr;
       const int ecol0 = item.n0 + half * 64, erow0 = item.m0 + q * 32;
       if (TEPI) {
@@ -476,7 +508,7 @@
         }
         __syncwarp();
       }
-      if (!TEPI && item.E != nullptr) {
+      if (!TEPI && !WIDE && item.E != nullptr) {
         auto prefetch_block = [&](const T2Item& it2) {
           const int prow = it2.m0 + q * 32 + lane;
           const int pcol = it2.n0 + half * 64;
@@ -490,35 +522,38 @@
         if (w == w0) prefetch_block(item);
         if (w + wstep < p.items) {
           int pidx2 = pidx;
-          prefetch_block(t2_item(p, w + wstep, pidx2, rank));
+          prefetch_block(t2_item<WIDE>(p, w + wstep, pidx2, rank));
         }
       }
       for (int kc0 = item.kb0; kc0 < item.kb1; kc0 += p.drain_kb, ++chain) {
-        const int j = chain & 1;
-        mbar_wait(tfull_bar(j), (chain >> 1) & 1);
+        const int j = WIDE ? 0 : chain & 1;
+        mbar_wait(tfull_bar(j), WIDE ? chain & 1 : (chain >> 1) & 1);
         tc_fence_after();
         const uint32_t cbase = lane_addr + (uint32_t)(2 * T2_BN * j);
         const float comp = 1.0f + p.comp * (float)(4 * (min(item.kb1, kc0 + p.drain_kb) - kc0));
-        uint32_t r[32];
-#pragma unroll
-        for (int part = 0; part < 4; ++part) {
-          T2_TMEM_LD32(r, cbase + (uint32_t)((part >> 1) * T2_BN + (part & 1) * 32));
+        uint32_t r[LDW];
+#pragma unroll
+        for (int part = 0; part < NPART; ++part) {
+          const int cross = part >= NPART / 2, cc = part % (NPART / 2);
+          const uint32_t taddr = cbase + (uint32_t)(cross * (WIDE ? 2 * T2_BN : T2_BN) + cc * LDW);
+          if constexpr (WIDE) T2_TMEM_LD16(r, taddr); else T2_TMEM_LD32(r, taddr);
           asm volatile("tcgen05.wait::ld.sync.aligned;" ::: "memory");
-          if (part == 3) {
+          if (part == NPART - 1 || (WIDE && part == NPART / 2 - 1)) {
+            const uint32_t bar = tempty_bar(WIDE ? cross : j);
             tc_fence_before();
             if (PAIR) {
               __syncwarp();
-              if (lane == 0) mbar_arrive_rank(tempty_bar(j), 0);
+              if (lane == 0) mbar_arrive_rank(bar, 0);
             } else {
-              mbar_arrive(tempty_bar(j));
+              mbar_arrive(bar);
             }
           }
-          if (part < 2) {
-#pragma unroll
-            for (int i = 0; i < 32; ++i) acc[(part & 1) * 32 + i] = fmaf(__uint_as_float(r[i]), comp, acc[(part & 1) * 32 + i]);
+          if (!cross) {
+#pragma unroll
+            for (int i = 0; i < LDW; ++i) acc[cc * LDW + i] = fmaf(__uint_as_float(r[i]), comp, acc[cc * LDW + i]);
           } else {
 #pragma unroll
-            for (int i = 0; i < 32; ++i) acc[(part & 1) * 32 + i] += __uint_as_float(r[i]);
+            for (int i = 0; i < LDW; ++i) acc[cc * LDW + i] += __uint_as_float(r[i]);
           }
         }
       }
@@ -579,7 +614,7 @@
       const bool do_relu = !to_slab && p.relu;
       const float* bias = to_slab ? nullptr : p.bias;
       const int row0 = item.m0 + q * 32;
-      if (item.E != nullptr && vec_ok && !add_c && !do_relu && !bias && (item.N & 3) == 0 && (item.lde & 3) == 0 &&
+      if (!WIDE && item.E != nullptr && vec_ok && !add_c && !do_relu && !bias && (item.N & 3) == 0 && (item.lde & 3) == 0 &&
           (reinterpret_cast<uintptr_t>(item.E) & 15) == 0) {
         const int c4 = (lane >> 3) * 4;
         const int rsub = lane & 7;
@@ -622,13 +657,13 @@
         continue;
       }
 #pragma unroll
-      for (int g = 0; g < 4; ++g) {
+      for (int g = 0; g < CW / 16; ++g) {
 #pragma unroll
         for (int jv = 0; jv < 16; jv += 4)
           *reinterpret_cast<float4*>(stg + lane * T2_EPI_ROW + jv) = make_float4(acc[g * 16 + jv], acc[g * 16 + jv + 1], acc[g * 16 + jv + 2], acc[g * 16 + jv + 3]);
         __syncwarp();
         const int c4 = (lane >> 3) * 4;
-        const int col = item.n0 + half * 64 + g * 16 + c4;
+        const int col = item.n0 + half * CW + g * 16 + c4;
         if (vec_ok && col + 3 < item.N) {
           const float4 bv = bias ? *reinterpret_cast<const float4*>(bias + col) : make_float4(0.f, 0.f, 0.f, 0.f);
 #pragma unroll
@@ -638,7 +673,7 @@
             if (row < item.M) {
               float4 v = *reinterpret_cast<const float4*>(stg + rr * T2_EPI_ROW + c4);
               v.x += bv.x; v.y += bv.y; v.z += bv.z; v.w += bv.w;
-              if (item.E) {
+              if (!WIDE && item.E) {
                 const float d = item.rowv[row];
                 const float* ep = item.E + (long long)row * item.lde + col;
                 float4 e4;
@@ -659,7 +694,7 @@
             for (int e = 0; e < 4; ++e) {
               if (row < item.M && col + e < item.N) {
                 float v = stg[rr * T2_EPI_ROW + c4 + e] + (bias ? bias[col + e] : 0.f);
-                if (item.E) v = item.E[(long long)row * item.lde + col + e] * (v - item.rowv[row]);
+                if (!WIDE && item.E) v = item.E[(long long)row * item.lde + col + e] * (v - item.rowv[row]);
                 float* dst = outp + (long long)row * ldo + col + e;
                 if (add_c) v += *dst;
                 if (do_relu) v = fmaxf(v, 0.f);
@@ -774,16 +809,23 @@
 }
 bool t2_tepi_operand_ok(const float* ptr, int64_t ld) { return ptr && (ld & 3) == 0 && (reinterpret_cast<uintptr_t>(ptr) & 15) == 0; }
 
+bool t2_wide_ok(int pair, int64_t n_min, int k_parts, bool any_e, int64_t wide_items) {
+  const char* e = getenv("DCB200_T2_WIDE");
+  if (e && e[0] == '0') return false;
+  return pair && n_min > T2_BN && k_parts == 1 && !any_e && wide_items >= sm_count() / 2;
+}
+
 int t2_launch(const CUtensorMap* mA, const CUtensorMap* mB, const CUtensorMap& mC, const T2Params& p, cudaStream_t st) {
   static DeviceOnce attr_set;
   if (attr_set.first()) {
-    DC_CUDA(cudaFuncSetAttribute(gemm_tc2_kernel<false, false>, cudaFuncAttributeMaxDynamicSharedMemorySize, T2_SMEM_BYTES));
-    DC_CUDA(cudaFuncSetAttribute(gemm_tc2_kernel<true, false>, cudaFuncAttributeMaxDynamicSharedMemorySize, T2_SMEM_BYTES));
-    DC_CUDA(cudaFuncSetAttribute(gemm_tc2_kernel<true, true>, cudaFuncAttributeMaxDynamicSharedMemorySize, T2_SMEM_BYTES));
+    DC_CUDA(cudaFuncSetAttribute(gemm_tc2_kernel<false, false, false>, cudaFuncAttributeMaxDynamicSharedMemorySize, T2_SMEM_BYTES));
+    DC_CUDA(cudaFuncSetAttribute(gemm_tc2_kernel<true, false, false>, cudaFuncAttributeMaxDynamicSharedMemorySize, T2_SMEM_BYTES));
+    DC_CUDA(cudaFuncSetAttribute(gemm_tc2_kernel<true, true, false>, cudaFuncAttributeMaxDynamicSharedMemorySize, T2_SMEM_BYTES));
+    DC_CUDA(cudaFuncSetAttribute(gemm_tc2_kernel<true, false, true>, cudaFuncAttributeMaxDynamicSharedMemorySize, T2_SMEM_BYTES));
   }
   if (!p.pair) {
     const int grid = p.items < sm_count() ? p.items : sm_count();
-    gemm_tc2_kernel<false, false><<<grid, T2_THREADS, T2_SMEM_BYTES, st>>>(mA[0], mA[1], mA[2], mA[3], mB[0], mB[1], mB[2], mB[3], mC, p);
+    gemm_tc2_kernel<false, false, false><<<grid, T2_THREADS, T2_SMEM_BYTES, st>>>(mA[0], mA[1], mA[2], mA[3], mB[0], mB[1], mB[2], mB[3], mC, p);
   } else {
     const int pairs = p.items < sm_count() / 2 ? p.items : sm_count() / 2;
     cudaLaunchConfig_t cfg{};
@@ -796,8 +838,8 @@
     at[0].val.clusterDim.x = 2; at[0].val.clusterDim.y = 1; at[0].val.clusterDim.z = 1;
     cfg.attrs = at;
     cfg.numAttrs = 1;
-    if (p.tepi) DC_CUDA(cudaLaunchKernelEx(&cfg, gemm_tc2_kernel<true, true>, mA[0], mA[1], mA[2], mA[3], mB[0], mB[1], mB[2], mB[3], mC, p));
-    else DC_CUDA(cudaLaunchKernelEx(&cfg, gemm_tc2_kernel<true, false>, mA[0], mA[1], mA[2], mA[3], mB[0], mB[1], mB[2], mB[3], mC, p));
+    auto kern = p.wide ? gemm_tc2_kernel<true, false, true> : p.tepi ? gemm_tc2_kernel<true, true, false> : gemm_tc2_kernel<true, false, false>;
+    DC_CUDA(cudaLaunchKernelEx(&cfg, kern, mA[0], mA[1], mA[2], mA[3], mB[0], mB[1], mB[2], mB[3], mC, p));
   }
   DC_LAUNCH_CHECK();
   return DC_OK;
@@ -838,9 +880,22 @@
   p.a_mn = transA ? 1 : 0;
   p.b_mn = transB ? 0 : 1;
   p.pair = t2_pair();
-  const uint32_t b_box_rows = p.pair ? T2_BN / 2 : T2_BN;
+  int64_t ktot = 0;
+  for (int s = 0; s < 4; ++s) {
+    p.kb_seg[s] = s < nseg ? (int)cdiv(segs[s].K, T2_BK) : (1 << 30);
+    if (s < nseg) ktot += cdiv(segs[s].K, T2_BK);
+  }
+  p.kb_total = (int)ktot;
+  p.M = (int)M; p.N = (int)N;
+  p.m_tiles = (int)cdiv(M, T2_BM);
+  p.k_parts = t2_k_parts(M, N, p.kb_total);
+  p.kb_per_part = (int)(cdiv(cdiv(p.kb_total, p.k_parts), T2_PART_KB) * T2_PART_KB);
+  p.k_parts = (int)cdiv(p.kb_total, p.kb_per_part);
+  p.wide = t2_wide_ok(p.pair, N, p.k_parts, false, cdiv(p.m_tiles, 2) * cdiv(N, 2 * T2_BN));
+  p.n_chunks = (int)cdiv(N, p.wide ? 2 * T2_BN : T2_BN);
+  p.items = (p.pair ? (p.m_tiles + 1) / 2 : p.m_tiles) * p.n_chunks * p.k_parts;
+  const uint32_t b_box_rows = p.pair && !p.wide ? T2_BN / 2 : T2_BN;
   CUtensorMap mA[4], mB[4];
-  int64_t ktot = 0;
   for (int s = 0; s < 4; ++s) {
     const int ss = s < nseg ? s : 0;
     const uint64_t K = (uint64_t)segs[ss].K;
@@ -854,17 +909,7 @@
     } else {
       if (int rc = make_map2(&mB[s], segs[ss].B, (uint64_t)N, K, (uint64_t)segs[ss].ldb, 32, CU_TENSOR_MAP_SWIZZLE_128B_ATOM_32B)) return rc;
     }
-    p.kb_seg[s] = s < nseg ? (int)cdiv(segs[s].K, T2_BK) : (1 << 30);
-    if (s < nseg) ktot += cdiv(segs[s].K, T2_BK);
-  }
-  p.kb_total = (int)ktot;
-  p.M = (int)M; p.N = (int)N;
-  p.m_tiles = (int)cdiv(M, T2_BM);
-  p.n_chunks = (int)cdiv(N, T2_BN);
-  p.k_parts = t2_k_parts(M, N, p.kb_total);
-  p.kb_per_part = (int)(cdiv(cdiv(p.kb_total, p.k_parts), T2_PART_KB) * T2_PART_KB);
-  p.k_parts = (int)cdiv(p.kb_total, p.kb_per_part);
-  p.items = (p.pair ? (p.m_tiles + 1) / 2 : p.m_tiles) * p.n_chunks * p.k_parts;
+  }
   p.drain_kb = t2_drain_kb(p.kb_total);
   p.C = C; p.ldc = ldc; p.bias = bias; p.relu = relu; p.accumulate = accumulate;
   p.raw_hi = 1;
@@ -876,7 +921,7 @@
     p.partial = reinterpret_cast<float*>((reinterpret_cast<uintptr_t>(workspace) + 255) & ~(uintptr_t)255);
   }
   CUtensorMap mC{};
-  p.tepi = t2_tepi_ok(p.pair, p.kb_total, p.k_parts, accumulate) && t2_tepi_operand_ok(C, ldc);
+  p.tepi = !p.wide && t2_tepi_ok(p.pair, p.kb_total, p.k_parts, accumulate) && t2_tepi_operand_ok(C, ldc);
   if (p.tepi)
     if (int rc = make_map2(&mC, C, (uint64_t)N, (uint64_t)M, (uint64_t)ldc, 32, CU_TENSOR_MAP_SWIZZLE_128B)) return rc;
   if (int rc = t2_launch(mA, mB, mC, p, st)) return rc;
@@ -913,20 +958,25 @@
   T2Problem* tab = reinterpret_cast<T2Problem*>(hbase);
   int* item_off = reinterpret_cast<int*>(hbase + tab_bytes);
   const int pair = t2_pair();
-  const uint32_t b_box_rows = pair ? T2_BN / 2 : T2_BN;
   int64_t items = 0;
   int64_t max_kb = 0;
   int64_t kb_all = 0;
   bool tepi_operands = true;
+  int64_t n_min = -1, wide_items = 0;
   for (int i = 0; i < count; ++i) {
     const dc_gemm_problem& q = probs[i];
     if (q.M <= 0 || q.N <= 0) continue;
     if (cdiv(q.K, T2_BK) > kb_all) kb_all = cdiv(q.K, T2_BK);
     if (!t2_tepi_operand_ok(q.C, q.ldc) || (q.E && !t2_tepi_operand_ok(q.E, q.lde))) tepi_operands = false;
+    if (n_min < 0 || q.N < n_min) n_min = q.N;
+    wide_items += cdiv(cdiv(q.M, T2_BM), 2) * cdiv(q.N, 2 * T2_BN);
   }
   bool any_e = false;
   for (int i = 0; i < count; ++i) any_e = any_e || probs[i].E != nullptr;
-  const int tepi = t2_tepi_ok(pair, kb_all, 1, accumulate) && tepi_operands && (t2_tepi_mode() != 3 || any_e);
+  const int wide = t2_wide_ok(pair, n_min, 1, any_e, wide_items);
+  const int tepi = !wide && t2_tepi_ok(pair, kb_all, 1, accumulate) && tepi_operands && (t2_tepi_mode() != 3 || any_e);
+  const uint32_t b_box_rows = pair && !wide ? T2_BN / 2 : T2_BN;
+  const int bn = wide ? 2 * T2_BN : T2_BN;
   for (int i = 0; i < count; ++i) {
     const dc_gemm_problem& q = probs[i];
     DC_REQUIRE(q.M >= 0 && q.N >= 0 && q.K >= 0, DC_EINVAL, "gemm_batched: negative size in problem %d", i);
@@ -958,7 +1008,7 @@
     }
     t.kb_total = (int)cdiv(q.K, T2_BK);
     if (t.kb_total > max_kb) max_kb = t.kb_total;
-    t.n_chunks = (int)cdiv(q.N, T2_BN);
+    t.n_chunks = (int)cdiv(q.N, bn);
     items += (pair ? cdiv(cdiv(q.M, T2_BM), 2) : cdiv(q.M, T2_BM)) * t.n_chunks;
     DC_REQUIRE(items < (1ll << 30), DC_ENOSUP, "gemm_batched: too many work items");
   }
@@ -976,6 +1026,7 @@
   p.b_mn = transB ? 0 : 1;
   p.k_parts = 1;
   p.pair = pair;
+  p.wide = wide;
   p.items = (int)items;
   p.drain_kb = t2_drain_kb(max_kb);
   p.relu = relu; p.accumulate = accumulate;
```

New measurement: 3193, median of 6. 13.1% higher.
